# djamahl99/findnpropagate

Measured on AMD Instinct MI355X. Metric: NuScenes scenes/s (30k pts, Transfusion voxel backbone), higher is better.
Workload: dtype bf16

## Files before the change

### findnpropagate_amd/csrc/sortedsweep.h

```cpp
#pragma once
#include "common.h"

namespace {

template <typename T> struct Vec16 {
    typedef T v8 __attribute__((ext_vector_type(8)));
    typedef T v4 __attribute__((ext_vector_type(4)));
};
typedef float f32x4_t __attribute__((ext_vector_type(4)));
__device__ __forceinline__ f32x4_t mfma16(Vec16<__bf16>::v8 a, Vec16<__bf16>::v8 b, f32x4_t c) {
    return __builtin_amdgcn_mfma_f32_16x16x32_bf16(a, b, c, 0, 0, 0);
}
__device__ __forceinline__ f32x4_t mfma16(Vec16<_Float16>::v8 a, Vec16<_Float16>::v8 b, f32x4_t c) {
    return __builtin_amdgcn_mfma_f32_16x16x32_f16(a, b, c, 0, 0, 0);
}
typedef float f32x4 __attribute__((ext_vector_type(4)));
typedef unsigned int u32x4 __attribute__((ext_vector_type(4)));

struct SortedRb {
    const int *perm;
    const unsigned *blockmask;
};

__device__ __forceinline__ void fnp_range_rows(int n, int range, int G, int &row_begin, int &row_end) {
    const long long nblk16 = (n + 15) >> 4;
    row_begin = (int)((nblk16 * range) / G) << 4;
    row_end = min(n, (int)((nblk16 * (range + 1)) / G) << 4);
}

struct XcdRows {
    int X0, X1, S;
};
__device__ __forceinline__ XcdRows fnp_xcd_rows(int n, int G, int xcd) {
    const int per = G >> 3, rem = G & 7;
    XcdRows x;
    x.S = per + (xcd < rem ? 1 : 0);
    x.X0 = x.X1 = 0;
    if (x.S > 0) {
        const int first = xcd < rem ? xcd * (per + 1) : rem * (per + 1) + (xcd - rem) * per;
        int t;
        fnp_range_rows(n, first, G, x.X0, t);
        fnp_range_rows(n, first + x.S - 1, G, t, x.X1);
    }
    return x;
}
__device__ __forceinline__ int fnp_tail_blocks(int rows_left, int S, int NW) {
    const int nb = (rows_left + 15) >> 4;
    return ((nb + S - 1) / S + NW - 1) / NW;
}

constexpr int kSortedNW = 8, kSortedMB = 3;

}

__attribute__((visibility("hidden"))) int fnp_launch_rows128(int dtype, const void *x, const void *w, const int *nbr, int nbr_stride, const int *n_out,
                                                             int cap, void *y, const float *scale, const float *shift, const void *residual, int relu,
                                                             const int *perm, const unsigned *blockmask, int grid, hipStream_t s);
```

### findnpropagate_amd/csrc/spconv.hip

```cpp
#include "rankgrid.h"
#include "sortedsweep.h"
#include <type_traits>

#ifndef FNP_ABLATE
#define FNP_ABLATE 0
#endif

namespace {

__device__ __forceinline__ float to_f32(float v) { return v; }
__device__ __forceinline__ float to_f32(__bf16 v) { return (float)v; }
__device__ __forceinline__ float to_f32(_Float16 v) { return (float)v; }
template <typename T> __device__ __forceinline__ T from_f32(float v);
template <> __device__ __forceinline__ float from_f32<float>(float v) { return v; }
template <> __device__ __forceinline__ __bf16 from_f32<__bf16>(float v) { return (__bf16)v; }
template <> __device__ __forceinline__ _Float16 from_f32<_Float16>(float v) { return (_Float16)v; }

template <typename TIn, typename TOut>
__global__ __launch_bounds__(256) void spconv_valu_kernel(const TIn *__restrict__ x, const TIn *__restrict__ w,
                                                          const int *__restrict__ nbr, int nbr_stride, int K,
                                                          const int *__restrict__ n_out, int cap,
                                                          TOut *__restrict__ y, const float *__restrict__ scale,
                                                          const float *__restrict__ shift,
                                                          const TOut *__restrict__ residual, int relu, int Cin, int Cout) {
// ... 821 lines not shown
                  const FusedRb *frb_in = nullptr, const SortedRb *srb_in = nullptr, int *grid_only = nullptr, const SplitOut *so_in = nullptr) {
    constexpr int NWX = NwOf<CIN, COUT, NWO>::value;
    constexpr int MB = NWO ? MfmaWg<CIN, COUT>::MB_SMALL : MfmaWg<CIN, COUT>::MB;
    using Cfg = MfmaCfg<CIN, COUT, KVOL>;
    auto kern = spconv_mfma_kernel<CIN, COUT, MB, KVOL, WIN, TOut, FUSED, TAct, SORTED, NWO>;
    constexpr int lds = Cfg::lds_bytes(NWX, MB, WIN) + Cfg::epi_bytes(NWX, WIN, sizeof(TOut) == 2) +
                        (FUSED ? NWX * 27 * MB * 16 * 4 : 0) + COUT * 8;
    FusedRb frb{};
    if (FUSED) {
        if (!frb_in) return FNP_ERR_ARG;
        frb = *frb_in;
    }
    SortedRb srb{nullptr, nullptr};
    if (SORTED && !grid_only) {
        if (!srb_in || !srb_in->perm || !srb_in->blockmask) return FNP_ERR_ARG;
        srb = *srb_in;
    }
    constexpr int wg_regs = MfmaOcc<CIN, COUT>::WAVES * 4 / NWX;
    constexpr int wg_per_cu = lds * wg_regs > 160 * 1024 ? 160 * 1024 / lds : wg_regs;
    static_assert(wg_per_cu >= 1 && lds * wg_per_cu <= 160 * 1024, "LDS budget of the resident workgroups");
    if (lds > 64 * 1024 && !grid_only) {
        static bool raised = false;
        if (!raised) {
            if (hipFuncSetAttribute(reinterpret_cast<const void *>(kern), hipFuncAttributeMaxDynamicSharedMemorySize, lds) != hipSuccess)
                return FNP_ERR_HIP;
            raised = true;
        }
    }
    const int tiles = fnp_divup(cap, NWX * MB * 16);
    const int resident = 256 * wg_per_cu;
    const int fine = fnp_divup(cap, NWX * 16);
    const int grid = tiles >= resident ? resident : (fine < resident ? fine : resident);
    if (grid_only) {
        *grid_only = grid;
        return FNP_OK;
    }
    hipLaunchKernelGGL(kern, dim3(grid), dim3(NWX * 64), lds, s, (const TAct *)x, x_bytes, (const TAct *)w,
                       nbr, nbr_stride, K, n_out, cap, (TOut *)y, scale, shift, (const TOut *)residual, relu, hints, frb, srb,
                       so_in ? *so_in : SplitOut{nullptr, nullptr, nullptr, 0});
    FNP_LAUNCH_CHECK();
    return FNP_OK;
}

template <int CIN, int COUT> struct HasWindow { static constexpr bool value = CIN == 64 && COUT == 64; };

template <int CIN, int COUT, typename TOut, typename TAct>
int launch_mfma(const void *x, int x_bytes, const void *w, const int *nbr, int nbr_stride, int K, const int *n_out,
                int cap, void *y, const float *scale, const float *shift, const void *residual, int relu, int hints,
                hipStream_t s, const SplitOut *so = nullptr) {
    if (K == 27) {
        if constexpr (HasWindow<CIN, COUT>::value) {
            if (hints & FNP_HINT_ROWS_RANKED)
                return launch_mfma_k<CIN, COUT, 27, true, TOut, false, TAct>(x, x_bytes, w, nbr, nbr_stride, K, n_out, cap, y, scale,
                                                                shift, residual, relu, hints, s, nullptr, nullptr, nullptr, so);
        }
        if constexpr (CIN == 128 && COUT == 128 && sizeof(TOut) == 2) {
            if (cap < 256 * MfmaWg<CIN, COUT>::NW * MfmaWg<CIN, COUT>::MB * 16)
                return launch_mfma_k<CIN, COUT, 27, false, TOut, false, TAct, false, 4>(x, x_bytes, w, nbr, nbr_stride, K, n_out, cap, y, scale, shift,
                                                                                        residual, relu, hints, s);
        }
        return launch_mfma_k<CIN, COUT, 27, false, TOut, false, TAct>(x, x_bytes, w, nbr, nbr_stride, K, n_out, cap, y, scale, shift,
                                                         residual, relu, hints, s, nullptr, nullptr, nullptr, so);
    }
    return launch_mfma_k<CIN, COUT, 0, false, TOut, false, TAct>(x, x_bytes, w, nbr, nbr_stride, K, n_out, cap, y, scale, shift, residual,
                                                    relu, hints, s, nullptr, nullptr, nullptr, so);
}

template <typename TIn, typename TOut>
int launch_valu(const void *x, const void *w, const int *nbr, int nbr_stride, int K, const int *n_out, int cap, void *y,
                const float *scale, const float *shift, const void *residual, int relu, int Cin, int Cout,
                hipStream_t s) {
    const int grid = fnp_grid_for((long long)cap * Cout, 256, 256 * 16);
    hipLaunchKernelGGL(HIP_KERNEL_NAME(spconv_valu_kernel<TIn, TOut>), dim3(grid), dim3(256), 0, s, (const TIn *)x,
                       (const TIn *)w, nbr, nbr_stride, K, n_out, cap, (TOut *)y, scale, shift, (const TOut *)residual,
                       relu, Cin, Cout);
    FNP_LAUNCH_CHECK();
    return FNP_OK;
}

constexpr int kSortThreads = 1024, kSortQ = 16;
__device__ __forceinline__ int fnp_zclass(unsigned m) {
    const bool lo = (m & 0x1ffu) != 0u, hi = (m & (0x1ffu << 18)) != 0u;
    return lo ? (hi ? 2 : 3) : (hi ? 1 : 0);
}
__global__ __launch_bounds__(256) void rowmask_kernel(const int *__restrict__ nbr, int nbr_stride, const int *__restrict__ n_out, int cap,
                                                      unsigned *__restrict__ rowmask) {
    const int n = min(*n_out, cap);
    for (int r = blockIdx.x * 256 + threadIdx.x; r < n; r += gridDim.x * 256) {
        unsigned m = 0u;
#pragma unroll
        for (int k = 0; k < 27; ++k) m |= (nbr[(size_t)k * nbr_stride + r] >= 0 ? 1u : 0u) << k;
        rowmask[r] = m;
    }
}
__global__ __launch_bounds__(kSortThreads) void classsort_place_kernel(const unsigned *__restrict__ rowmask, const int *__restrict__ n_out, int cap,
                                                                        int G, int tile_rows, int NW, int *__restrict__ perm,
                                                                        unsigned *__restrict__ blockmask) {
    constexpr int NWV = kSortThreads / 64;
    __shared__ unsigned long long wtot[NWV];
    const int n = min(*n_out, cap), tid = threadIdx.x, lane = tid & 63, wave = tid >> 6;
    const XcdRows xr = fnp_xcd_rows(n, G, blockIdx.y);
    if (xr.S == 0 || xr.X0 >= xr.X1) return;
    const int round_rows = xr.S * tile_rows, full = (xr.X1 - xr.X0) / round_rows;
    for (int i = blockIdx.x; i <= full; i += gridDim.x) {
        const int b = xr.X0 + i * round_rows, e = min(xr.X1, b + round_rows);
        if (b >= e) break;
        const int q = (e - b + kSortThreads - 1) / kSortThreads, r0 = b + tid * q;
        for (int j = (b >> 4) + tid; j < ((e + 15) >> 4); j += kSortThreads) blockmask[j] = 0u;
        unsigned m[kSortQ];
        unsigned long long cnt = 0ull;
#pragma unroll
        for (int u = 0; u < kSortQ; ++u) {
            m[u] = 0u;
            if (u < q && r0 + u < e) {
                m[u] = rowmask[r0 + u];
                cnt += 1ull << (16 * fnp_zclass(m[u]));
            }
        }
        unsigned long long v = cnt;
#pragma unroll
        for (int d = 1; d < 64; d <<= 1) {
            const unsigned long long t = __shfl_up(v, d);
            if (lane >= d) v += t;
        }
        if (lane == 63) wtot[wave] = v;
        __syncthreads();
        unsigned long long woff = 0ull, grand = 0ull;
#pragma unroll
        for (int wv = 0; wv < NWV; ++wv) {
            const unsigned long long t = wtot[wv];
            if (wv < wave) woff += t;
            grand += t;
        }
        const unsigned long long excl = v - cnt + woff;
        int run[4];
        const int t0 = (int)(grand & 0xffffu), t1 = (int)((grand >> 16) & 0xffffu), t2 = (int)((grand >> 32) & 0xffffu);
        run[0] = (int)(excl & 0xffffu);
        run[1] = t0 + (int)((excl >> 16) & 0xffffu);
        run[2] = t0 + t1 + (int)((excl >> 32) & 0xffffu);
        run[3] = t0 + t1 + t2 + (int)((excl >> 48) & 0xffffu);
#pragma unroll
        for (int u = 0; u < kSortQ; ++u) {
            if (u < q && r0 + u < e) {
                const int c = fnp_zclass(m[u]);
                const int pos = b + (c == 0 ? run[0]++ : c == 1 ? run[1]++ : c == 2 ? run[2]++ : run[3]++);
                perm[pos] = r0 + u;
                atomicOr(&blockmask[pos >> 4], m[u]);
            }
        }
        __syncthreads();
    }
}

template <typename TAct, typename TOut>
int dispatch_16(const void *x, long long n_in, const void *w, const int *nbr, int nbr_stride, int K, const int *n_out, int cap,
                  void *y, const float *scale, const float *shift, const void *residual, int relu, int hints, int Cin,
                  int Cout, hipStream_t s, const SplitOut *so = nullptr) {
    const long long xb = n_in * Cin * 2;
    const bool fits = xb > 0 && xb < 0x7fffffffll;
#define FNP_CASE(CI, CO)                                                                                       \
    if (fits && Cin == CI && Cout == CO)                                                                       \
        return launch_mfma<CI, CO, TOut, TAct>(x, (int)xb, w, nbr, nbr_stride, K, n_out, cap, y, scale, shift, residual,\
                                         relu, hints, s, so);
    FNP_CASE(16, 16)
    FNP_CASE(16, 32)
    FNP_CASE(32, 32)
    FNP_CASE(32, 64)
    FNP_CASE(64, 64)
    FNP_CASE(64, 128)
    FNP_CASE(128, 128)
    FNP_CASE(32, 16)
    FNP_CASE(64, 32)
    FNP_CASE(128, 64)
#undef FNP_CASE
    if (so) return FNP_ERR_ARG;
    return launch_valu<TAct, TOut>(x, w, nbr, nbr_stride, K, n_out, cap, y, scale, shift, residual, relu, Cin, Cout, s);
}

}

#ifdef FNP_MFMA_STAMP
extern "C" int fnp_debug_mfma_stamps(unsigned long long *out8) {
    if (hipMemcpyFromSymbol(out8, HIP_SYMBOL(g_mfma_stamps), sizeof(unsigned long long) * 8) != hipSuccess) return FNP_ERR_HIP;
    unsigned long long zero[8] = {0};
    if (hipMemcpyToSymbol(HIP_SYMBOL(g_mfma_stamps), zero, sizeof(zero)) != hipSuccess) return FNP_ERR_HIP;
    return FNP_OK;
}
#endif

int fnp_spconv_forward_f32_mfma(const void *feat_in, long long n_in_rows, const void *weight, const int *nbr, int nbr_stride,
                                int K, const int *n_out, int cap_out, void *feat_out, const float *scale, const float *shift,
                                const void *residual, int relu, int wperm, int Cin, int Cout, hipStream_t s);

extern "C" int fnp_spconv_forward(const void *feat_in, int in_dtype, int n_in_rows, const void *weight, const int *nbr,
                                  int nbr_stride, int K, const int *n_out, int cap_out, void *feat_out, int out_dtype,
                                  const float *scale, const float *shift, const void *residual, int relu, int hints,
                                  int Cin, int Cout, fnp_stream_t stream) {
    hipStream_t s = (hipStream_t)stream;
    if (!feat_in || !weight || !nbr || !n_out || !feat_out || K <= 0 || Cin <= 0 || Cout <= 0 || cap_out <= 0 ||
        nbr_stride < cap_out || n_in_rows <= 0)
        return FNP_ERR_ARG;
    if ((scale == nullptr) != (shift == nullptr)) return FNP_ERR_ARG;
    if (in_dtype == FNP_F32 && Cout == 16 && Cin <= 8 && (size_t)K * Cin * 16 * 4 <= 60000) {
        if (out_dtype == FNP_F32)
            return launch_first<float>(feat_in, weight, nbr, nbr_stride, K, n_out, cap_out, feat_out, scale, shift,
                                       residual, relu, Cin, s);
        if (out_dtype == FNP_BF16)
            return launch_first<__bf16>(feat_in, weight, nbr, nbr_stride, K, n_out, cap_out, feat_out, scale, shift,
                                        residual, relu, Cin, s);
        if (out_dtype == FNP_F16)
            return launch_first<_Float16>(feat_in, weight, nbr, nbr_stride, K, n_out, cap_out, feat_out, scale, shift,
                                          residual, relu, Cin, s);
        return FNP_ERR_ARG;
    }
    if (in_dtype == FNP_F32) {
        if (out_dtype == FNP_F32 && !(hints & FNP_HINT_VALU)) {
            const int rc = fnp_spconv_forward_f32_mfma(feat_in, n_in_rows, weight, nbr, nbr_stride, K, n_out, cap_out, feat_out,
                                                       scale, shift, residual, relu, (hints & FNP_HINT_W_PERMUTED) != 0, Cin, Cout, s);
            if (rc != FNP_ERR_ARG) return rc;
        }
        if (hints & FNP_HINT_W_PERMUTED) return FNP_ERR_ARG;
        if (out_dtype == FNP_F32)
            return launch_valu<float, float>(feat_in, weight, nbr, nbr_stride, K, n_out, cap_out, feat_out, scale, shift,
                                             residual, relu, Cin, Cout, s);
        if (out_dtype == FNP_BF16)
            return launch_valu<float, __bf16>(feat_in, weight, nbr, nbr_stride, K, n_out, cap_out, feat_out, scale,
                                              shift, residual, relu, Cin, Cout, s);
        if (out_dtype == FNP_F16)
            return launch_valu<float, _Float16>(feat_in, weight, nbr, nbr_stride, K, n_out, cap_out, feat_out, scale,
                                                shift, residual, relu, Cin, Cout, s);
        return FNP_ERR_ARG;
    }
    if (in_dtype == FNP_BF16) {
        if (out_dtype == FNP_BF16)
            return dispatch_16<__bf16, __bf16>(feat_in, n_in_rows, weight, nbr, nbr_stride, K, n_out, cap_out, feat_out, scale, shift,
                                               residual, relu, hints, Cin, Cout, s);
        if (out_dtype == FNP_F32)
            return dispatch_16<__bf16, float>(feat_in, n_in_rows, weight, nbr, nbr_stride, K, n_out, cap_out, feat_out, scale, shift,
                                              residual, relu, hints, Cin, Cout, s);
        return FNP_ERR_ARG;
    }
    if (in_dtype == FNP_F16) {
        if (out_dtype == FNP_F16)
            return dispatch_16<_Float16, _Float16>(feat_in, n_in_rows, weight, nbr, nbr_stride, K, n_out, cap_out, feat_out, scale,
                                                   shift, residual, relu, hints, Cin, Cout, s);
        if (out_dtype == FNP_F32)
            return dispatch_16<_Float16, float>(feat_in, n_in_rows, weight, nbr, nbr_stride, K, n_out, cap_out, feat_out, scale, shift,
                                                residual, relu, hints, Cin, Cout, s);
        return FNP_ERR_ARG;
    }
    return FNP_ERR_ARG;
}

extern "C" int fnp_spconv_forward_split(const void *feat_in, int in_dtype, int n_in_rows, const void *weight, const int *nbr, int nbr_stride,
                                        int K, const int *n_out, int cap_out, float *feat_out, const float *scale, const float *shift,
                                        const float *residual, const void *addend, int relu, int hints, int Cin, int Cout, void *out_hi,
                                        void *out_lo, fnp_stream_t stream) {
    hipStream_t s = (hipStream_t)stream;
    if (!feat_in || !weight || !nbr || !n_out || !out_hi || !out_lo || K <= 0 || Cin <= 0 || Cout <= 0 || cap_out <= 0 ||
        nbr_stride < cap_out || n_in_rows <= 0 || (scale == nullptr) != (shift == nullptr))
        return FNP_ERR_ARG;
    if ((((uintptr_t)out_hi | (uintptr_t)out_lo | (uintptr_t)addend) & 7) || ((uintptr_t)feat_out & 15)) return FNP_ERR_ARG;
    const SplitOut so{addend, out_hi, out_lo, relu};
    if (in_dtype == FNP_BF16)
        return dispatch_16<__bf16, float>(feat_in, n_in_rows, weight, nbr, nbr_stride, K, n_out, cap_out, feat_out, scale, shift, residual, 0, hints,
                                          Cin, Cout, s, &so);
    if (in_dtype == FNP_F16)
        return dispatch_16<_Float16, float>(feat_in, n_in_rows, weight, nbr, nbr_stride, K, n_out, cap_out, feat_out, scale, shift, residual, 0, hints,
                                            Cin, Cout, s, &so);
    return FNP_ERR_ARG;
}

extern "C" int fnp_spconv_forward_strided(const void *feat_in, int in_dtype, int n_in_rows, const void *weight,
                                          const fnp_rankgrid *in_grid, const fnp_conv_geom *geom, const int *out_coords,
                                          const int *n_out, int cap_out, void *feat_out, int out_dtype, const float *scale,
                                          const float *shift, int relu, int Cin, int Cout, fnp_stream_t stream) {
    hipStream_t s = (hipStream_t)stream;
    if (!feat_in || !weight || !geom || !out_coords || !n_out || !feat_out || cap_out <= 0 || n_in_rows <= 0 ||
        !fnp_rg_valid(in_grid))
        return FNP_ERR_ARG;
    if ((scale == nullptr) != (shift == nullptr)) return FNP_ERR_ARG;
    if ((in_dtype != FNP_BF16 && in_dtype != FNP_F16) || out_dtype != in_dtype) return FNP_ERR_ARG;
    for (int d = 0; d < 3; ++d)
        if (geom->ksize[d] != 3 || geom->stride[d] <= 0 || geom->padding[d] < 0) return FNP_ERR_ARG;
    if (in_grid->D != geom->in_shape[0] || in_grid->H != geom->in_shape[1] || in_grid->W != geom->in_shape[2]) return FNP_ERR_ARG;
    const long long xb = (long long)n_in_rows * Cin * 2;
    if (xb <= 0 || xb >= 0x7fffffffll) return FNP_ERR_ARG;
    FusedRb frb;
    frb.gi = fnp_rg_view(in_grid);
    for (int d = 0; d < 3; ++d) {
        frb.s[d] = geom->stride[d];
        frb.p[d] = geom->padding[d];
    }
    frb.out_coords = out_coords;
    frb.ell_rec = nullptr;
    frb.ell_cap = 0;
#define FNP_FCASE(CI, CO)                                                                                                   \
    if (Cin == CI && Cout == CO) {                                                                                          \
        if (in_dtype == FNP_F16)                                                                                            \
            return launch_mfma_k<CI, CO, 27, false, _Float16, true, _Float16>(feat_in, (int)xb, weight, nullptr, cap_out, 27, n_out, \
                                                                              cap_out, feat_out, scale, shift, nullptr, relu, 0, s, &frb); \
        return launch_mfma_k<CI, CO, 27, false, __bf16, true>(feat_in, (int)xb, weight, nullptr, cap_out, 27, n_out, cap_out, feat_out, \
                                                              scale, shift, nullptr, relu, 0, s, &frb);                     \
    }
    FNP_FCASE(16, 32)
    FNP_FCASE(32, 64)
    FNP_FCASE(64, 128)
#undef FNP_FCASE
    return FNP_ERR_ARG;
}

extern "C" int fnp_spconv_forward_ell_mfma(const void *feat_in, int in_dtype, int n_in_rows, const void *weight, const void *records, int cap_rows,
// ... 115 lines not shown
```

### findnpropagate_amd/csrc/spconv_rows128.hip

```cpp
#include "sortedsweep.h"
#include <type_traits>

#ifndef FNP_R128_ABLATE
#define FNP_R128_ABLATE 0
#endif

namespace {

__device__ uint4 g_rows128_zero[8];

template <int I> __device__ __forceinline__ int fnp_row_share(int v) { return __builtin_amdgcn_update_dpp(0, v, 0x150 + I, 0xf, 0xf, false); }
template <int I, int N, typename F> __device__ __forceinline__ void fnp_static_for(F &&f) {
    if constexpr (I < N) {
        f(std::integral_constant<int, I>{});
        fnp_static_for<I + 1, N>(f);
    }
}
typedef __attribute__((address_space(1))) const void *fnp_gptr;
typedef __attribute__((address_space(3))) void *fnp_lptr;

#define FNP_VMCNT(N) asm volatile("s_waitcnt vmcnt(%0)" ::"n"(N) : "memory")
#define FNP_LGKMCNT0() asm volatile("s_waitcnt lgkmcnt(0)" ::: "memory")

constexpr int kR128NW = kSortedNW, kR128MB = kSortedMB, kR128NT = kR128NW * 64;
constexpr int kR128Slab = 128 * 128, kR128Ring = 3;
constexpr int kR128RowBuf = kR128MB * 16 * 128;
constexpr int kR128RowsOff = kR128Ring * kR128Slab, kR128EntOff = kR128RowsOff + 2 * kR128NW * kR128RowBuf;
constexpr int kR128Lds = kR128EntOff + kR128NW * 2 * 256;
static_assert(kR128Lds == 148 * 1024 && kR128Lds <= 160 * 1024, "slab ring + two row buffers + entry slots");
static_assert(kR128RowBuf >= 16 * (128 * 2 + 16), "the epilogue's transpose strip aliases the wave's first row buffer");

template <typename TAct>
__global__ __launch_bounds__(kR128NT, 2) void spconv_rows128_kernel(const TAct *__restrict__ x, const TAct *__restrict__ w, const int *__restrict__ nbr,
                                                                    int nbr_stride, const int *__restrict__ n_out, int cap, TAct *__restrict__ y,
                                                                    const float *__restrict__ scale, const float *__restrict__ shift,
                                                                    const TAct *__restrict__ residual, int relu, SortedRb srb) {
    using bf16x8 = typename Vec16<TAct>::v8;
    using bf16x4 = typename Vec16<TAct>::v4;
    constexpr int C = 128, NB = 8, NBH = 4, NW = kR128NW, MB = kR128MB, ROWS_PER_WG = NW * MB * 16;
    constexpr int NSLAB = (FNP_R128_ABLATE & 2) ? 0 : 2;
    extern __shared__ __attribute__((aligned(16))) unsigned char fnp_smem[];
    const int n = min(*n_out, cap);
    const int tid = threadIdx.x, lane = tid & 63, wave = __builtin_amdgcn_readfirstlane(tid >> 6);
    const int l15 = lane & 15, q = lane >> 4;
    const int r8 = lane >> 3, c8 = lane & 7;
    unsigned char *const rowbuf = fnp_smem + kR128RowsOff + wave * kR128RowBuf;
    unsigned char *const entbuf = fnp_smem + kR128EntOff + wave * 512;

    const int G = gridDim.x, xcd = blockIdx.x & 7, slot = blockIdx.x >> 3;
    const XcdRows xr = fnp_xcd_rows(n, G, xcd);
    const int row_begin = xr.X0, row_end = xr.X1, xslots = xr.S;
    if (row_begin >= row_end) return;

    unsigned foff[2];
#pragma unroll
    for (int ksl = 0; ksl < 2; ++ksl) foff[ksl] = (unsigned)l15 * 128u + ((unsigned)((ksl * 4 + q) ^ ((l15 >> 1) & 7)) << 4);
    unsigned wsrc[2];
#pragma unroll
    for (int j = 0; j < 2; ++j) {
        const int wr = (j * 8 + wave) * 8 + r8;
        wsrc[j] = (unsigned)wr * 256u + ((unsigned)(c8 ^ ((wr >> 1) & 7)) << 4);
    }
    auto dma_slab_piece = [&](int koffset, int half, int ring, int j) {
        const unsigned char *wk = reinterpret_cast<const unsigned char *>(w) + (size_t)koffset * (C * C * 2) + half * 128;
        __builtin_amdgcn_global_load_lds((fnp_gptr)(wk + wsrc[j]), (fnp_lptr)(fnp_smem + ring * kR128Slab + (j * 8 + wave) * 1024), 16, 0, 0);
    };

    struct TileSt {
        int Kt, kl, erow;
    };
    const int c16 = lane & 15, r4 = lane >> 4;
    auto tile_epos = [&](int tile_base, int mbt) -> int { return tile_base + wave * (mbt * 16) + 8 * (c16 >> 1) + 2 * r4 + (c16 & 1); };
    auto tile_loads = [&](int tile_base, int mbt, unsigned &m, int &erow) {
        const int nbt = min(NW * mbt, (row_end - tile_base + 15) >> 4);
        m = lane < nbt ? srb.blockmask[(tile_base >> 4) + lane] : 0u;
        erow = srb.perm[min(tile_epos(tile_base, mbt), row_end - 1)];
    };
    auto tile_state = [&](unsigned m, int erow) -> TileSt {
        TileSt st;
        st.erow = erow;
        st.kl = 0;
#pragma unroll
        for (int d = 32; d >= 1; d >>= 1) m |= (unsigned)__shfl_xor((int)m, d);
        m = (unsigned)__builtin_amdgcn_readfirstlane((int)m) & 0x7ffffffu;
        if (m == 0u) m = 1u << 13;
        st.Kt = __popc(m);
        int cnt = 0;
#pragma unroll
        for (int pbit = 0; pbit < 27; ++pbit) {
            if ((m >> pbit) & 1u) {
                if (lane >= cnt) st.kl = pbit;
                ++cnt;
            }
        }
        return st;
    };
    auto dma_ent_of = [&](const TileSt &st, int i, int es) {
        const int ko = __builtin_amdgcn_readlane(st.kl, i < st.Kt ? i : st.Kt - 1);
        __builtin_amdgcn_global_load_lds((fnp_gptr)(nbr + (size_t)ko * nbr_stride + st.erow), (fnp_lptr)(entbuf + es * 256), 4, 0, 0);
    };

    auto run_tile = [&](auto mbt_tag, const int tile_base, const TileSt st, const int next_base, const int next_mbt) __attribute__((always_inline)) -> TileSt {
        constexpr int MBT = decltype(mbt_tag)::value, NI = MBT * 2;
        constexpr int NROW = (FNP_R128_ABLATE & 4) ? 0 : NI;
        const int row0 = tile_base + wave * (MBT * 16);
        const int Kt = st.Kt, kl = st.kl;
        auto koff = [&](int i) -> int { return __builtin_amdgcn_readlane(kl, i < Kt ? i : Kt - 1); };
        const bool ehas = c16 < 2 * NI && tile_epos(tile_base, MBT) < row_end;
        auto dma_ent = [&](int i, int es) { dma_ent_of(st, i, es); };
        auto read_ent = [&](int es) -> int { return *reinterpret_cast<const int *>(entbuf + es * 256 + lane * 4); };
        auto dma_row_piece = [&](int ev, auto half_tag, auto ic) {
            constexpr int half = decltype(half_tag)::value, ii = decltype(ic)::value;
            const int e0 = fnp_row_share<2 * ii>(ev), e1 = fnp_row_share<2 * ii + 1>(ev);
            const int er = (FNP_R128_ABLATE & 8) ? -1 : (lane & 8) ? e1 : e0;
            const int sw = ((ii & 1) << 2) | (r8 >> 1);
            const unsigned char *src = er >= 0 ? reinterpret_cast<const unsigned char *>(x) + (size_t)er * 256 + (half * 128 + ((c8 ^ sw) << 4))
                                               : reinterpret_cast<const unsigned char *>(g_rows128_zero) + (c8 << 4);
            __builtin_amdgcn_global_load_lds((fnp_gptr)src, (fnp_lptr)(rowbuf + half * (NW * kR128RowBuf) + ii * 1024), 16, 0, 0);
        };
        auto dma_piece = [&](auto pc, auto half_tag, const int k, const int ev, const int ring_s2) {
            constexpr int p = decltype(pc)::value, half = decltype(half_tag)::value;
            if constexpr (p < NROW) dma_row_piece(ev, half_tag, pc);
            else if constexpr (p < NROW + NSLAB) dma_slab_piece(koff(k + 1), half, ring_s2, p - NROW);
            else if constexpr (p == NROW + NSLAB && half == 0) dma_ent(k + 2, k & 1);
        };
        bf16x8 xb[2][MBT];
        auto read_xb = [&](int half, int k) {
            const unsigned char *rb = rowbuf + half * (NW * kR128RowBuf);
#pragma unroll
            for (int ksl = 0; ksl < 2; ++ksl)
#pragma unroll
                for (int mb = 0; mb < MBT; ++mb) {
                    u32x4 t = u32x4{(unsigned)k, 0u, 0u, 0u};
                    if (!(FNP_R128_ABLATE & 4)) t = *reinterpret_cast<const u32x4 *>(rb + mb * 2048 + foff[ksl]);
                    xb[ksl][mb] = *reinterpret_cast<const bf16x8 *>(&t);
                }
        };

        f32x4 acc[NB][MBT];
#pragma unroll
        for (int nb = 0; nb < NB; ++nb)
#pragma unroll
            for (int mb = 0; mb < MBT; ++mb) acc[nb][mb] = (f32x4){0.f, 0.f, 0.f, 0.f};

        auto step = [&](auto half_tag, const int k, const bool more, const int e_next, const int ring_s, const int ring_s2) {
            constexpr int half = decltype(half_tag)::value;
            constexpr int NG = 4, SLOTS = NG * MBT, NP = NROW + NSLAB + 1;
            const unsigned char *wk = fnp_smem + ring_s * kR128Slab;
            const int ev = ehas ? e_next : -1;
            bf16x8 wa[2][NBH];
            auto read_wa = [&](auto gc) {
                constexpr int g = decltype(gc)::value;
#pragma unroll
                for (int j = 0; j < NBH; ++j) {
                    u32x4 t = u32x4{(unsigned)k, 1u, 0u, 0u};
                    if (!(FNP_R128_ABLATE & 2)) t = *reinterpret_cast<const u32x4 *>(wk + ((g & 1) * NBH + j) * 2048 + foff[g >> 1]);
                    wa[g & 1][j] = *reinterpret_cast<const bf16x8 *>(&t);
                }
            };
            read_wa(std::integral_constant<int, 0>{});
            FNP_LGKMCNT0();
            __builtin_amdgcn_sched_barrier(0);
            fnp_static_for<0, NG>([&](auto gc) {
                constexpr int g = decltype(gc)::value;
                if constexpr (g + 1 < NG) read_wa(std::integral_constant<int, g + 1>{});
                fnp_static_for<0, MBT>([&](auto mc) {
                    constexpr int mb = decltype(mc)::value, sl = g * MBT + mb;
#pragma unroll
                    for (int j = 0; j < NBH; ++j) {
                        if (FNP_R128_ABLATE & 1) asm volatile("" ::"v"(wa[g & 1][j]), "v"(xb[g >> 1][mb]));
                        else acc[(g & 1) * NBH + j][mb] = mfma16(wa[g & 1][j], xb[g >> 1][mb], acc[(g & 1) * NBH + j][mb]);
                    }
                    if (more) {
                        fnp_static_for<sl * NP / SLOTS, (sl + 1) * NP / SLOTS>([&](auto pc) { dma_piece(pc, half_tag, k, ev, ring_s2); });
                    }
                    __builtin_amdgcn_sched_barrier(0);
                });
            });
            if (FNP_R128_ABLATE & 16) {
            } else if (more) FNP_VMCNT(NROW + NSLAB + (half == 0 ? 1 : 0));
            else FNP_VMCNT(0);
            if (half == 0 || more) read_xb(half ^ 1, k);
            __builtin_amdgcn_sched_barrier(0);
            __builtin_amdgcn_s_barrier();
            __builtin_amdgcn_sched_barrier(0);
        };

        FNP_LGKMCNT0();
        FNP_VMCNT(0);
        __builtin_amdgcn_sched_barrier(0);
        {
            const int e0 = read_ent(0);
            FNP_LGKMCNT0();
            __builtin_amdgcn_sched_barrier(0);
            const int ev0 = ehas ? e0 : -1;
            fnp_static_for<0, NROW>([&](auto ic) { dma_row_piece(ev0, std::integral_constant<int, 0>{}, ic); });
            fnp_static_for<0, NSLAB>([&](auto jc) { dma_slab_piece(koff(0), 0, 0, decltype(jc)::value); });
            fnp_static_for<0, NROW>([&](auto ic) { dma_row_piece(ev0, std::integral_constant<int, 1>{}, ic); });
            fnp_static_for<0, NSLAB>([&](auto jc) { dma_slab_piece(koff(0), 1, 1, decltype(jc)::value); });
        }
        __builtin_amdgcn_sched_barrier(0);
        FNP_VMCNT(NROW + NSLAB);
        read_xb(0, 0);
        __builtin_amdgcn_sched_barrier(0);
        __builtin_amdgcn_s_barrier();
        __builtin_amdgcn_sched_barrier(0);
        int ring = 0;
        for (int k = 0; k < Kt; ++k) {
            const bool more = k + 1 < Kt;
            const int r1 = ring == 2 ? 0 : ring + 1, r2 = r1 == 2 ? 0 : r1 + 1;
            const int e_next = read_ent((k + 1) & 1);
            step(std::integral_constant<int, 0>{}, k, more, e_next, ring, r2);
            step(std::integral_constant<int, 1>{}, k, more, e_next, r1, ring);
            ring = r2;
        }

        constexpr int EH = 16, LPR = C / 8, SPI = 64 / LPR, NRD = EH / SPI, ES = C * 2 + 16;
        unsigned char *const eb = rowbuf;
        const int wsite = lane / LPR, wchunk = lane % LPR;
        u32x4 rs_all[MBT][NRD];
        int orow[MBT][NRD];
        unsigned nm = 0u;
        int nerow = 0;
        if (next_mbt) tile_loads(next_base, next_mbt, nm, nerow);
#pragma unroll
        for (int mb = 0; mb < MBT; ++mb)
#pragma unroll
            for (int i = 0; i < NRD; ++i) {
                const int r = row0 + mb * 16 + i * SPI + wsite;
                orow[mb][i] = srb.perm[r < row_end ? r : row_end - 1];
            }
        TileSt nst{1, 13, 0};
        if (next_mbt) {
            nst = tile_state(nm, nerow);
            dma_ent_of(nst, 0, 0);
            dma_ent_of(nst, 1, 1);
        }
        if (residual) {
#pragma unroll
            for (int mb = 0; mb < MBT; ++mb)
#pragma unroll
                for (int i = 0; i < NRD; ++i)
                    rs_all[mb][i] = *reinterpret_cast<const u32x4 *>(residual + (size_t)orow[mb][i] * C + wchunk * 8);
        }
#pragma unroll
        for (int mb = 0; mb < MBT; ++mb) {
            const int rb = row0 + mb * 16;
            if (residual) {
#pragma unroll
                for (int i = 0; i < NRD; ++i) *reinterpret_cast<u32x4 *>(eb + (i * SPI + wsite) * ES + wchunk * 16) = rs_all[mb][i];
            }
#pragma unroll
            for (int nb = 0; nb < NB; ++nb) {
                const int c0 = nb * 16 + q * 4;
                float v[4];
#pragma unroll
                for (int j = 0; j < 4; ++j) v[j] = acc[nb][mb][j];
                if (scale) {
                    const float4 s4 = *reinterpret_cast<const float4 *>(scale + c0);
                    const float4 h4 = *reinterpret_cast<const float4 *>(shift + c0);
                    v[0] = v[0] * s4.x + h4.x; v[1] = v[1] * s4.y + h4.y; v[2] = v[2] * s4.z + h4.z; v[3] = v[3] * s4.w + h4.w;
                }
                bf16x4 *slotp = reinterpret_cast<bf16x4 *>(eb + l15 * ES + c0 * 2);
                if (residual) {
                    const bf16x4 t = *slotp;
#pragma unroll
                    for (int j = 0; j < 4; ++j) v[j] = v[j] + (float)t[j];
                }
                if (relu) {
#pragma unroll
                    for (int j = 0; j < 4; ++j) v[j] = v[j] < 0.f ? 0.f : v[j];
                }
                *slotp = bf16x4{(TAct)v[0], (TAct)v[1], (TAct)v[2], (TAct)v[3]};
            }
#pragma unroll
            for (int i = 0; i < NRD; ++i) {
                const int r = rb + i * SPI + wsite;
                const u32x4 t = *reinterpret_cast<const u32x4 *>(eb + (i * SPI + wsite) * ES + wchunk * 16);
                if (r < row_end) *reinterpret_cast<u32x4 *>(y + (size_t)orow[mb][i] * C + wchunk * 8) = t;
            }
        }
        return nst;
    };

    const int round_rows = xslots * ROWS_PER_WG;
    const int full = (row_end - row_begin) / round_rows;
    const int left0 = row_begin + full * round_rows;
    int tper = fnp_tail_blocks(row_end - left0, xslots, NW);
    const int tail_base = left0 + slot * (NW * tper * 16);
    if (tail_base >= row_end) tper = 0;
    const int rot = (xslots * 3 + 4) >> 3;
    auto full_base = [&](int t) -> int { return row_begin + t * round_rows + ((slot + t * rot) % xslots) * ROWS_PER_WG; };
    if (full == 0 && tper == 0) return;
    TileSt st;
    {
        unsigned m0;
        int erow0;
        tile_loads(full ? full_base(0) : tail_base, full ? MB : tper, m0, erow0);
        st = tile_state(m0, erow0);
        dma_ent_of(st, 0, 0);
        dma_ent_of(st, 1, 1);
    }
    for (int t = 0; t < full; ++t) {
        const bool last = t + 1 == full;
        st = run_tile(std::integral_constant<int, MB>{}, full_base(t), st, last ? tail_base : full_base(t + 1), last ? tper : MB);
    }
    if (tper == 3) run_tile(std::integral_constant<int, 3>{}, tail_base, st, 0, 0);
    if (tper == 2) run_tile(std::integral_constant<int, 2>{}, tail_base, st, 0, 0);
    if (tper == 1) run_tile(std::integral_constant<int, 1>{}, tail_base, st, 0, 0);
}

template <typename TAct>
int launch_rows128(const void *x, const void *w, const int *nbr, int nbr_stride, const int *n_out, int cap, void *y, const float *scale,
                   const float *shift, const void *residual, int relu, const SortedRb &srb, int grid, hipStream_t s) {
    auto kern = spconv_rows128_kernel<TAct>;
    static bool raised = false;
    if (!raised) {
        if (hipFuncSetAttribute(reinterpret_cast<const void *>(kern), hipFuncAttributeMaxDynamicSharedMemorySize, kR128Lds) != hipSuccess) return FNP_ERR_HIP;
        raised = true;
    }
    hipLaunchKernelGGL(kern, dim3(grid), dim3(kR128NT), kR128Lds, s, (const TAct *)x, (const TAct *)w, nbr, nbr_stride, n_out, cap, (TAct *)y, scale, shift,
                       (const TAct *)residual, relu, srb);
    FNP_LAUNCH_CHECK();
    return FNP_OK;
}

}

int fnp_launch_rows128(int dtype, const void *x, const void *w, const int *nbr, int nbr_stride, const int *n_out, int cap, void *y, const float *scale,
                       const float *shift, const void *residual, int relu, const int *perm, const unsigned *blockmask, int grid, hipStream_t s) {
    const SortedRb srb{perm, blockmask};
    if (dtype == FNP_BF16) return launch_rows128<__bf16>(x, w, nbr, nbr_stride, n_out, cap, y, scale, shift, residual, relu, srb, grid, s);
    if (dtype == FNP_F16) return launch_rows128<_Float16>(x, w, nbr, nbr_stride, n_out, cap, y, scale, shift, residual, relu, srb, grid, s);
    return FNP_ERR_ARG;
}
```

Before: 13740.

## Add output-stationary K=3 128-channel spconv kernel and peel last rows128 step

Result: faster. 14120, median of 6 (+2.8%).

```diff
diff --git a/findnpropagate_amd/csrc/sortedsweep.h b/findnpropagate_amd/csrc/sortedsweep.h
--- a/findnpropagate_amd/csrc/sortedsweep.h
+++ b/findnpropagate_amd/csrc/sortedsweep.h
@@ -56,3 +56,7 @@
 __attribute__((visibility("hidden"))) int fnp_launch_rows128(int dtype, const void *x, const void *w, const int *nbr, int nbr_stride, const int *n_out,
                                                              int cap, void *y, const float *scale, const float *shift, const void *residual, int relu,
                                                              const int *perm, const unsigned *blockmask, int grid, hipStream_t s);
+
+__attribute__((visibility("hidden"))) int fnp_launch_out128(int in_dtype, int out_f32, const void *x, int x_bytes, const void *w, const int *nbr,
+                                                            int nbr_stride, const int *n_out, int cap, void *y, const float *scale, const float *shift,
+                                                            int relu, hipStream_t s);
diff --git a/findnpropagate_amd/csrc/spconv.hip b/findnpropagate_amd/csrc/spconv.hip
--- a/findnpropagate_amd/csrc/spconv.hip
+++ b/findnpropagate_amd/csrc/spconv.hip
@@ -997,12 +997,20 @@
     }
 }
 
+#ifndef FNP_OUT128_MIN_CAP
+#define FNP_OUT128_MIN_CAP (256 * 8 * 64)
+#endif
+constexpr int kOut128MinCap = FNP_OUT128_MIN_CAP;
+
 template <typename TAct, typename TOut>
 int dispatch_16(const void *x, long long n_in, const void *w, const int *nbr, int nbr_stride, int K, const int *n_out, int cap,
                   void *y, const float *scale, const float *shift, const void *residual, int relu, int hints, int Cin,
                   int Cout, hipStream_t s, const SplitOut *so = nullptr) {
     const long long xb = n_in * Cin * 2;
     const bool fits = xb > 0 && xb < 0x7fffffffll;
+    if (fits && K == 3 && Cin == 128 && Cout == 128 && !residual && !so && cap >= kOut128MinCap)
+        return fnp_launch_out128(std::is_same<TAct, __bf16>::value ? FNP_BF16 : FNP_F16, sizeof(TOut) == 4, x, (int)xb, w, nbr, nbr_stride, n_out, cap, y,
+                                 scale, shift, relu, s);
 #define FNP_CASE(CI, CO)                                                                                       \
     if (fits && Cin == CI && Cout == CO)                                                                       \
         return launch_mfma<CI, CO, TOut, TAct>(x, (int)xb, w, nbr, nbr_stride, K, n_out, cap, y, scale, shift, residual,\
diff --git a/findnpropagate_amd/csrc/spconv_out128.hip b/findnpropagate_amd/csrc/spconv_out128.hip
--- /dev/null
+++ b/findnpropagate_amd/csrc/spconv_out128.hip
@@ -0,0 +1,214 @@
+#include "sortedsweep.h"
+#include <type_traits>
+
+namespace {
+
+constexpr int kO128C = 128;
+constexpr int kO128K = 3;
+constexpr int kO128NW = 8, kO128NT = kO128NW * 64;
+constexpr int kO128MB = 2;
+constexpr int kO128CH = kO128C / 8;
+constexpr int kO128Slab = kO128C * kO128CH;
+constexpr int kO128SlabBytes = kO128K * kO128Slab * 16;
+constexpr int kO128StripBytes = 16 * (kO128C * 2 + 16);
+static_assert(8 * (kO128C * 4 + 16) <= kO128StripBytes, "f32 pass of eight rows fits the strip");
+constexpr int kO128Lds = kO128SlabBytes + kO128NW * kO128StripBytes + 2 * kO128C * 4;
+static_assert(kO128Lds <= 160 * 1024, "LDS of a CU");
+
+template <typename TAct, typename TOut>
+__global__ __launch_bounds__(kO128NT, 2) void spconv_out128_kernel(const TAct *__restrict__ x, int x_bytes, const TAct *__restrict__ w,
+                                                                   const int *__restrict__ nbr, int nbr_stride, const int *__restrict__ n_out, int cap,
+                                                                   TOut *__restrict__ y, const float *__restrict__ scale, const float *__restrict__ shift,
+                                                                   int relu) {
+    using bf16x8 = typename Vec16<TAct>::v8;
+    using bf16x4 = typename Vec16<TAct>::v4;
+    static_assert(sizeof(TOut) == 4 || std::is_same<TOut, TAct>::value, "16-bit outputs have the activation type");
+    constexpr int C = kO128C, K = kO128K, CH = kO128CH, SLAB = kO128Slab, MB = kO128MB;
+    constexpr int KS = C / 32;
+    constexpr int NB = C / 16;
+    constexpr int NBH = 4;
+
+    extern __shared__ __attribute__((aligned(16))) unsigned char o128_smem[];
+    uint4 *const wl = reinterpret_cast<uint4 *>(o128_smem);
+    float *const ss_lds = reinterpret_cast<float *>(o128_smem + kO128SlabBytes + kO128NW * kO128StripBytes);
+
+    const int n = min(*n_out, cap);
+    const int tid = threadIdx.x;
+    const int lane = tid & 63, wave = tid >> 6;
+    const int l15 = lane & 15, q = lane >> 4;
+
+#define FNP_O128_POS(row, chunk) ((row) * CH + ((chunk) ^ ((row) & (CH - 1))))
+    for (int p = tid; p < K * SLAB; p += kO128NT) {
+        const int kk = p / SLAB, r = p % SLAB;
+        wl[kk * SLAB + FNP_O128_POS(r / CH, r % CH)] = reinterpret_cast<const uint4 *>(w)[p];
+    }
+    for (int c = tid; c < 2 * C; c += kO128NT) ss_lds[c] = scale ? (c < C ? scale[c] : shift[c - C]) : (c < C ? 1.f : 0.f);
+    __syncthreads();
+
+    int row_begin, row_end;
+    fnp_range_rows(n, (int)fnp_xcd_block() * kO128NW + wave, (int)gridDim.x * kO128NW, row_begin, row_end);
+    if (row_begin >= row_end) return;
+
+    int aoff[KS];
+#pragma unroll
+    for (int ks = 0; ks < KS; ++ks) aoff[ks] = FNP_O128_POS(l15, ks * 4 + q);
+#undef FNP_O128_POS
+
+    const __amdgpu_buffer_rsrc_t xrsrc = __builtin_amdgcn_make_buffer_rsrc((void *)x, 0, x_bytes, 0x00020000);
+    auto row_off = [&](int id, int r) -> unsigned {
+        return (id < 0 || r >= row_end) ? 0x80000000u : (unsigned)id * (unsigned)(C * 2) + (unsigned)q * 16u;
+    };
+    auto gather = [&](unsigned roff, int ks) -> bf16x8 {
+        const u32x4 v = __builtin_amdgcn_raw_buffer_load_b128(xrsrc, roff + (unsigned)ks * 64u, 0, 0);
+        return *reinterpret_cast<const bf16x8 *>(&v);
+    };
+    auto ent_raw = [&](int k, int r) -> int { return nbr[(size_t)k * nbr_stride + (r < row_end ? r : row_end - 1)]; };
+
+    unsigned char *const eb = o128_smem + kO128SlabBytes + wave * kO128StripBytes;
+    constexpr int ES = C * (int)sizeof(TOut) + 16;
+    constexpr int EH = sizeof(TOut) == 2 ? 16 : 8;
+    constexpr int LPR = C * (int)sizeof(TOut) / 16;
+    constexpr int SPI = 64 / LPR;
+    constexpr int NRD = EH / SPI;
+    const int wsite = lane / LPR, wchunk = lane % LPR;
+
+    bf16x8 xb[K][KS][MB];
+    int eq[K][MB];
+#pragma unroll
+    for (int k = 0; k < K; ++k)
+#pragma unroll
+        for (int mb = 0; mb < MB; ++mb) eq[k][mb] = ent_raw(k, row_begin + MB * 16 + mb * 16 + l15);
+    unsigned ro0[K][MB];
+#pragma unroll
+    for (int k = 0; k < K; ++k)
+#pragma unroll
+        for (int mb = 0; mb < MB; ++mb) {
+            const int r = row_begin + mb * 16 + l15;
+            ro0[k][mb] = row_off(ent_raw(k, r), r);
+        }
+    __builtin_amdgcn_sched_barrier(0);
+#pragma unroll
+    for (int k = 0; k < K; ++k) {
+#pragma unroll
+        for (int ks = 1; ks < KS; ks += 2) {
+#pragma unroll
+            for (int mb = 0; mb < MB; ++mb) {
+                xb[k][ks - 1][mb] = gather(ro0[k][mb], ks - 1);
+                xb[k][ks][mb] = gather(ro0[k][mb], ks);
+            }
+            __builtin_amdgcn_sched_barrier(0);
+        }
+    }
+
+    for (int row0 = row_begin; row0 < row_end; row0 += MB * 16) {
+        int en[K][MB];
+#pragma unroll
+        for (int k = 0; k < K; ++k)
+#pragma unroll
+            for (int mb = 0; mb < MB; ++mb) en[k][mb] = ent_raw(k, row0 + 2 * MB * 16 + mb * 16 + l15);
+        f32x4 acc[NB][MB];
+#pragma unroll
+        for (int nb = 0; nb < NB; ++nb)
+#pragma unroll
+            for (int mb = 0; mb < MB; ++mb) acc[nb][mb] = (f32x4){0.f, 0.f, 0.f, 0.f};
+#pragma unroll
+        for (int k = 0; k < K; ++k) {
+            const uint4 *wk = wl + k * SLAB;
+#pragma unroll
+            for (int ks = 0; ks < KS; ++ks) {
+#pragma unroll
+                for (int h = 0; h < NB; h += NBH) {
+                    bf16x8 wa[NBH];
+#pragma unroll
+                    for (int j = 0; j < NBH; ++j) {
+                        const uint4 t = wk[aoff[ks] + (h + j) * 16 * CH];
+                        wa[j] = *reinterpret_cast<const bf16x8 *>(&t);
+                    }
+#pragma unroll
+                    for (int mb = 0; mb < MB; ++mb)
+#pragma unroll
+                        for (int j = 0; j < NBH; ++j) acc[h + j][mb] = mfma16(wa[j], xb[k][ks][mb], acc[h + j][mb]);
+                }
+                if (ks & 1) {
+#pragma unroll
+                    for (int mb = 0; mb < MB; ++mb) {
+                        const int r = row0 + MB * 16 + mb * 16 + l15;
+                        const unsigned ro = row_off(eq[k][mb], r);
+                        xb[k][ks - 1][mb] = gather(ro, ks - 1);
+                        xb[k][ks][mb] = gather(ro, ks);
+                    }
+                }
+                __builtin_amdgcn_sched_barrier(0);
+            }
+        }
+#pragma unroll
+        for (int k = 0; k < K; ++k)
+#pragma unroll
+            for (int mb = 0; mb < MB; ++mb) eq[k][mb] = en[k][mb];
+
+#pragma unroll
+        for (int mb = 0; mb < MB; ++mb) {
+            if (row0 + mb * 16 >= row_end) break;
+#pragma unroll
+            for (int h = 0; h < 16 / EH; ++h) {
+                const int rb = row0 + mb * 16 + h * EH;
+                const bool mine = EH == 16 || (l15 / EH) == h;
+#pragma unroll
+                for (int nb = 0; nb < NB; ++nb) {
+                    const int c0 = nb * 16 + q * 4;
+                    float v[4];
+#pragma unroll
+                    for (int j = 0; j < 4; ++j) v[j] = acc[nb][mb][j];
+                    if (scale) {
+                        const float4 s4 = *reinterpret_cast<const float4 *>(ss_lds + c0);
+                        const float4 h4 = *reinterpret_cast<const float4 *>(ss_lds + C + c0);
+                        v[0] = v[0] * s4.x + h4.x; v[1] = v[1] * s4.y + h4.y; v[2] = v[2] * s4.z + h4.z; v[3] = v[3] * s4.w + h4.w;
+                    }
+                    if (relu) {
+#pragma unroll
+                        for (int j = 0; j < 4; ++j) v[j] = v[j] < 0.f ? 0.f : v[j];
+                    }
+                    if (mine) {
+                        unsigned char *slot = eb + (l15 % EH) * ES + c0 * (int)sizeof(TOut);
+                        if constexpr (sizeof(TOut) == 2) *reinterpret_cast<bf16x4 *>(slot) = bf16x4{(TAct)v[0], (TAct)v[1], (TAct)v[2], (TAct)v[3]};
+                        else *reinterpret_cast<f32x4 *>(slot) = (f32x4){v[0], v[1], v[2], v[3]};
+                    }
+                }
+#pragma unroll
+                for (int i = 0; i < NRD; ++i) {
+                    const int r = rb + i * SPI + wsite;
+                    const u32x4 t = *reinterpret_cast<const u32x4 *>(eb + (i * SPI + wsite) * ES + wchunk * 16);
+                    if (r < row_end) *reinterpret_cast<u32x4 *>(reinterpret_cast<unsigned char *>(y) + (size_t)r * (C * sizeof(TOut)) + wchunk * 16) = t;
+                }
+            }
+        }
+    }
+}
+
+template <typename TAct, typename TOut>
+int launch_out128(const void *x, int x_bytes, const void *w, const int *nbr, int nbr_stride, const int *n_out, int cap, void *y, const float *scale,
+                  const float *shift, int relu, hipStream_t s) {
+    auto kern = spconv_out128_kernel<TAct, TOut>;
+    static bool raised = false;
+    if (!raised) {
+        if (hipFuncSetAttribute(reinterpret_cast<const void *>(kern), hipFuncAttributeMaxDynamicSharedMemorySize, kO128Lds) != hipSuccess) return FNP_ERR_HIP;
+        raised = true;
+    }
+    hipLaunchKernelGGL(kern, dim3(256), dim3(kO128NT), kO128Lds, s, (const TAct *)x, x_bytes, (const TAct *)w, nbr, nbr_stride, n_out, cap, (TOut *)y, scale,
+                       shift, relu);
+    FNP_LAUNCH_CHECK();
+    return FNP_OK;
+}
+
+}
+
+int fnp_launch_out128(int in_dtype, int out_f32, const void *x, int x_bytes, const void *w, const int *nbr, int nbr_stride, const int *n_out, int cap, void *y,
+                      const float *scale, const float *shift, int relu, hipStream_t s) {
+    if (in_dtype == FNP_BF16)
+        return out_f32 ? launch_out128<__bf16, float>(x, x_bytes, w, nbr, nbr_stride, n_out, cap, y, scale, shift, relu, s)
+                       : launch_out128<__bf16, __bf16>(x, x_bytes, w, nbr, nbr_stride, n_out, cap, y, scale, shift, relu, s);
+    if (in_dtype == FNP_F16)
+        return out_f32 ? launch_out128<_Float16, float>(x, x_bytes, w, nbr, nbr_stride, n_out, cap, y, scale, shift, relu, s)
+                       : launch_out128<_Float16, _Float16>(x, x_bytes, w, nbr, nbr_stride, n_out, cap, y, scale, shift, relu, s);
+    return FNP_ERR_ARG;
+}
diff --git a/findnpropagate_amd/csrc/spconv_rows128.hip b/findnpropagate_amd/csrc/spconv_rows128.hip
--- a/findnpropagate_amd/csrc/spconv_rows128.hip
+++ b/findnpropagate_amd/csrc/spconv_rows128.hip
@@ -143,8 +143,9 @@
 #pragma unroll
             for (int mb = 0; mb < MBT; ++mb) acc[nb][mb] = (f32x4){0.f, 0.f, 0.f, 0.f};
 
-        auto step = [&](auto half_tag, const int k, const bool more, const int e_next, const int ring_s, const int ring_s2) {
+        auto step = [&](auto half_tag, auto more_tag, const int k, const int e_next, const int ring_s, const int ring_s2) __attribute__((always_inline)) {
             constexpr int half = decltype(half_tag)::value;
+            constexpr bool more = decltype(more_tag)::value;
             constexpr int NG = 4, SLOTS = NG * MBT, NP = NROW + NSLAB + 1;
             const unsigned char *wk = fnp_smem + ring_s * kR128Slab;
             const int ev = ehas ? e_next : -1;
@@ -205,14 +206,23 @@
         __builtin_amdgcn_sched_barrier(0);
         __builtin_amdgcn_s_barrier();
         __builtin_amdgcn_sched_barrier(0);
+        int prow = 0;
+        unsigned nm = 0u;
+        int nerow = 0;
         int ring = 0;
-        for (int k = 0; k < Kt; ++k) {
-            const bool more = k + 1 < Kt;
+        for (int k = 0; k + 1 < Kt; ++k) {
             const int r1 = ring == 2 ? 0 : ring + 1, r2 = r1 == 2 ? 0 : r1 + 1;
             const int e_next = read_ent((k + 1) & 1);
-            step(std::integral_constant<int, 0>{}, k, more, e_next, ring, r2);
-            step(std::integral_constant<int, 1>{}, k, more, e_next, r1, ring);
+            step(std::integral_constant<int, 0>{}, std::true_type{}, k, e_next, ring, r2);
+            step(std::integral_constant<int, 1>{}, std::true_type{}, k, e_next, r1, ring);
             ring = r2;
+        }
+        {
+            const int r1 = ring == 2 ? 0 : ring + 1, r2 = r1 == 2 ? 0 : r1 + 1;
+            if (next_mbt) tile_loads(next_base, next_mbt, nm, nerow);
+            prow = srb.perm[min(row0 + lane, row_end - 1)];
+            step(std::integral_constant<int, 0>{}, std::false_type{}, Kt - 1, 0, ring, r2);
+            step(std::integral_constant<int, 1>{}, std::false_type{}, Kt - 1, 0, r1, ring);
         }
 
         constexpr int EH = 16, LPR = C / 8, SPI = 64 / LPR, NRD = EH / SPI, ES = C * 2 + 16;
@@ -220,16 +230,10 @@
         const int wsite = lane / LPR, wchunk = lane % LPR;
         u32x4 rs_all[MBT][NRD];
         int orow[MBT][NRD];
-        unsigned nm = 0u;
-        int nerow = 0;
-        if (next_mbt) tile_loads(next_base, next_mbt, nm, nerow);
 #pragma unroll
         for (int mb = 0; mb < MBT; ++mb)
 #pragma unroll
-            for (int i = 0; i < NRD; ++i) {
-                const int r = row0 + mb * 16 + i * SPI + wsite;
-                orow[mb][i] = srb.perm[r < row_end ? r : row_end - 1];
-            }
+            for (int i = 0; i < NRD; ++i) orow[mb][i] = __shfl(prow, mb * 16 + i * SPI + wsite);
         TileSt nst{1, 13, 0};
         if (next_mbt) {
             nst = tile_state(nm, nerow);
```
